# zhaoshan2/pangu-pytorch

Measured on AMD Instinct MI355X. Metric: forward steps/sec (721x1440x13pl) per MI355X, higher is better.
Workload: dtype f32; 1 GPU; PanguModel fp32 forward, 1 sample/GPU, input (1,5,13,721,1440)+(1,4,721,1440), depths 2-6-6-2, dims 192/384, random-init weights (BASELINE configs[1]); parallelism=dp1

## Files before the change

pangu-pytorch_amd/csrc/gemm_ln_f32_split.hip:

```cpp
#include "ln_epilogue_f32.h"
#include "split_f32.h"

namespace {

using namespace pangu_split;

template <int WMW, int WNW, int NST, bool ROWS, bool HAS_BIAS>
__global__ __launch_bounds__(64 * WMW * WNW, WMW * WNW == 8 ? 1 : 2) void gemm_ln_residual_f32_split_kernel(
    const float* __restrict__ A, int lda, const unsigned char* __restrict__ image, const float* __restrict__ bias,
    const float* __restrict__ shortcut, int lds_sc, const float* __restrict__ gamma, const float* __restrict__ beta,
    float* __restrict__ C, int ldc, int M, int K, float branch_scale) {
  using Tile = SplitTile<WMW, WNW, NST, ROWS>;
  __shared__ __attribute__((aligned(16))) unsigned char smem[Tile::SMEM];
  const int m0 = blockIdx.x * Tile::BM;
  f32x16 acc[Tile::RB][Tile::CB];
  split_main_loop<WMW, WNW, NST, ROWS>(smem, A, lda, image, M, Tile::BN, K, m0, 0, acc);
  if constexpr (ROWS)
    pangu_ln::ln_residual_epilogue_rows<WMW, WNW, HAS_BIAS>(smem, acc, bias, shortcut, lds_sc, gamma, beta, C, ldc, M, m0,
                                                            branch_scale);
  else
    pangu_ln::ln_residual_epilogue<WMW, WNW, HAS_BIAS, false>(smem, acc, bias, shortcut, lds_sc, gamma, beta, C, ldc, M, m0,
                                                             branch_scale);
}

template <int WMW, int WNW, int NST, bool ROWS>
int launch_ln_split(hipStream_t s, const float* A, int lda, const unsigned char* image, const float* bias, const float* shortcut,
                    int lds, const float* gamma, const float* beta, float* out, int ldo, int M, int K, float branch_scale) {
  constexpr int BM = SplitTile<WMW, WNW, NST, ROWS>::BM;
  dim3 g((M + BM - 1) / BM), blk(64 * WMW * WNW);
  if (bias)
    hipLaunchKernelGGL((gemm_ln_residual_f32_split_kernel<WMW, WNW, NST, ROWS, true>), g, blk, 0, s, A, lda, image, bias, shortcut,
                       lds, gamma, beta, out, ldo, M, K, branch_scale);
  else
    hipLaunchKernelGGL((gemm_ln_residual_f32_split_kernel<WMW, WNW, NST, ROWS, false>), g, blk, 0, s, A, lda, image, bias, shortcut,
                       lds, gamma, beta, out, ldo, M, K, branch_scale);
  return pangu_launch_status();
}

}

extern "C" int pangu_linear_ln_residual_fwd_split(pangu_stream_t stream, const float* A, int lda, const void* image,
                                                  const float* bias, const float* shortcut, int lds, const float* gamma,
                                                  const float* beta, float* out, int ldo, int M, int N, int K,
                                                  float branch_scale) {
  if (!A || !image || !shortcut || !gamma || !beta || !out) return PANGU_E_NULL;
  if (M <= 0 || K <= 0 || (K % BK) != 0 || lda < K || (lda & 3) || ldo < N || (ldo & 3) || lds < N || (lds & 3))
    return PANGU_E_SHAPE;
  if (N != 192 && N != 384) return PANGU_E_SHAPE;
  if (!pangu_fits_u32(M, lda, 4) || !pangu_fits_u32(M, ldo, 4) || !pangu_fits_u32(M, lds, 4) ||
      (long long)N * K * 6 >= 0xFFFFFFFFll)
    return PANGU_E_RANGE;
  hipStream_t s = (hipStream_t)stream;
  const unsigned char* img = reinterpret_cast<const unsigned char*>(image);
  if (N == 192) return launch_ln_split<2, 2, 3, false>(s, A, lda, img, bias, shortcut, lds, gamma, beta, out, ldo, M, K, branch_scale);
  if (K < 1536) return launch_ln_split<1, 4, 2, false>(s, A, lda, img, bias, shortcut, lds, gamma, beta, out, ldo, M, K, branch_scale);
  return launch_ln_split<2, 2, 2, true>(s, A, lda, img, bias, shortcut, lds, gamma, beta, out, ldo, M, K, branch_scale);
}
```

pangu-pytorch_amd/csrc/ln_epilogue_f32.h:

```cpp
#pragma once
#include "common.h"

namespace pangu_ln {

__device__ inline float oct_sum(float v) {
  v += __builtin_bit_cast(float, __builtin_amdgcn_update_dpp(0, __builtin_bit_cast(int, v), 0xB1, 0xF, 0xF, true));
  v += __builtin_bit_cast(float, __builtin_amdgcn_update_dpp(0, __builtin_bit_cast(int, v), 0x4E, 0xF, 0xF, true));
  v += __builtin_bit_cast(float, __builtin_amdgcn_update_dpp(0, __builtin_bit_cast(int, v), 0x141, 0xF, 0xF, true));
  return v;
}

template <int WMW, int WNW, bool HAS_BIAS, bool PIN_COL>
__device__ __forceinline__ void ln_residual_epilogue(unsigned char* smem, const f32x16 (&acc)[2][3], const float* __restrict__ bias,
                                                     const float* __restrict__ shortcut, int lds_sc,
                                                     const float* __restrict__ gamma, const float* __restrict__ beta,
                                                     float* __restrict__ C, int ldc, int M, int m0, float branch_scale) {
  constexpr int NW = WMW * WNW;
  constexpr int BN = 96 * WNW;
  constexpr int EP_LD = 36;
  constexpr float INV_C = 1.0f / BN;
  const int lane = threadIdx.x & 63;
  const int wave = __builtin_amdgcn_readfirstlane(threadIdx.x >> 6);
  const int wm = wave / WNW, wn = wave % WNW;
  const int lr = lane & 31, lh = lane >> 5;
  float* ep = reinterpret_cast<float*>(smem) + wave * (32 * EP_LD);
  float* stats = reinterpret_cast<float*>(smem) + NW * (32 * EP_LD);
  const int er = lane >> 3, ec = (lane & 7) * 4;
  const __amdgpu_buffer_rsrc_t c_rsrc = __builtin_amdgcn_make_buffer_rsrc(
      C, 0, (int)(((size_t)(M - 1) * ldc + BN) * sizeof(float)), 0x00020000);
  const __amdgpu_buffer_rsrc_t s_rsrc = __builtin_amdgcn_make_buffer_rsrc(
      const_cast<float*>(shortcut), 0, (int)(((size_t)(M - 1) * lds_sc + BN) * sizeof(float)), 0x00020000);
#pragma unroll
  for (int i = 0; i < 2; ++i) {
    f32x4 y[3][4];
    float s[4] = {0.f, 0.f, 0.f, 0.f}, q[4] = {0.f, 0.f, 0.f, 0.f};
#pragma unroll
    for (int j = 0; j < 3; ++j) {
      int col = wn * 96 + j * 32 + ec;
      if (PIN_COL) asm volatile("" : "+v"(col));
      f32x4 bv = {0.f, 0.f, 0.f, 0.f};
      if (HAS_BIAS) bv = *reinterpret_cast<const f32x4*>(bias + col);
#pragma unroll
      for (int r = 0; r < 16; ++r) ep[((r & 3) + 8 * (r >> 2) + 4 * lh) * EP_LD + lr] = acc[i][j][r];
#pragma unroll
      for (int it = 0; it < 4; ++it) {
        f32x4 v = *reinterpret_cast<const f32x4*>(&ep[(er + 8 * it) * EP_LD + ec]);
        v += bv;
        y[j][it] = v;
        s[it] += (v[0] + v[1]) + (v[2] + v[3]);
        q[it] += (v[0] * v[0] + v[1] * v[1]) + (v[2] * v[2] + v[3] * v[3]);
      }
    }
#pragma unroll
    for (int it = 0; it < 4; ++it) {
      const float ss = oct_sum(s[it]), qq = oct_sum(q[it]);
      if ((lane & 7) == 0) {
        float* st = stats + (((wm * WNW + wn) * 64) + i * 32 + er + 8 * it) * 2;
        st[0] = ss;
        st[1] = qq;
      }
    }
    __syncthreads();
    float mean[4], rstd[4];
#pragma unroll
    for (int it = 0; it < 4; ++it) {
      const int rloc = i * 32 + er + 8 * it;
      float ts = 0.f, tq = 0.f;
#pragma unroll
      for (int w = 0; w < WNW; ++w) {
        const float* st = stats + ((wm * WNW + w) * 64 + rloc) * 2;
        ts += st[0];
        tq += st[1];
      }
      mean[it] = ts * INV_C;
      rstd[it] = rsqrtf(fmaxf(tq * INV_C - mean[it] * mean[it], 0.f) + LN_EPS);
    }
#pragma unroll
    for (int j = 0; j < 3; ++j) {
      int col = wn * 96 + j * 32 + ec;
      if (PIN_COL) asm volatile("" : "+v"(col));
      const f32x4 gm = *reinterpret_cast<const f32x4*>(gamma + col);
      const f32x4 bt = *reinterpret_cast<const f32x4*>(beta + col);
#pragma unroll
      for (int it = 0; it < 4; ++it) {
        const unsigned row = (unsigned)(m0 + wm * 64 + i * 32 + er + 8 * it);
        const f32x4 sc = __builtin_bit_cast(
            f32x4, __builtin_amdgcn_raw_buffer_load_b128(s_rsrc, (int)((row * (unsigned)lds_sc + (unsigned)col) * 4u), 0, 0));
        const f32x4 v = sc + branch_scale * ((y[j][it] - mean[it]) * rstd[it] * gm + bt);
        __builtin_amdgcn_raw_buffer_store_b128(__builtin_bit_cast(u32x4, v), c_rsrc,
                                               (int)((row * (unsigned)ldc + (unsigned)col) * 4u), 0, 0);
      }
    }
  }
}

template <int WMW, int WNW, bool HAS_BIAS>
__device__ __forceinline__ void ln_residual_epilogue_rows(unsigned char* smem, const f32x16 (&acc)[1][6],
                                                          const float* __restrict__ bias, const float* __restrict__ shortcut,
                                                          int lds_sc, const float* __restrict__ gamma,
                                                          const float* __restrict__ beta, float* __restrict__ C, int ldc, int M,
                                                          int m0, float branch_scale) {
  constexpr int NW = WMW * WNW;
  constexpr int BN = 192 * WNW;
  constexpr int NG = 2 * WNW;
  constexpr int EP_LD = 36;
  constexpr float INV_C = 1.0f / BN;
  const int lane = threadIdx.x & 63;
  const int wave = __builtin_amdgcn_readfirstlane(threadIdx.x >> 6);
  const int wm = wave / WNW, wn = wave % WNW;
  const int lr = lane & 31, lh = lane >> 5;
  float* ep = reinterpret_cast<float*>(smem) + wave * (32 * EP_LD);
  float* stats = reinterpret_cast<float*>(smem) + NW * (32 * EP_LD);
  const int er = lane >> 3, ec = (lane & 7) * 4;
  const __amdgpu_buffer_rsrc_t c_rsrc = __builtin_amdgcn_make_buffer_rsrc(
      C, 0, (int)(((size_t)(M - 1) * ldc + BN) * sizeof(float)), 0x00020000);
  const __amdgpu_buffer_rsrc_t s_rsrc = __builtin_amdgcn_make_buffer_rsrc(
      const_cast<float*>(shortcut), 0, (int)(((size_t)(M - 1) * lds_sc + BN) * sizeof(float)), 0x00020000);
  f32x4 y[6][4];
#pragma unroll
  for (int g = 0; g < 2; ++g) {
    float s[4] = {0.f, 0.f, 0.f, 0.f}, q[4] = {0.f, 0.f, 0.f, 0.f};
#pragma unroll
    for (int jj = 0; jj < 3; ++jj) {
      const int j = 3 * g + jj;
      const int col = wn * 192 + j * 32 + ec;
      f32x4 bv = {0.f, 0.f, 0.f, 0.f};
      if (HAS_BIAS) bv = *reinterpret_cast<const f32x4*>(bias + col);
#pragma unroll
      for (int r = 0; r < 16; ++r) ep[((r & 3) + 8 * (r >> 2) + 4 * lh) * EP_LD + lr] = acc[0][j][r];
#pragma unroll
      for (int it = 0; it < 4; ++it) {
        f32x4 v = *reinterpret_cast<const f32x4*>(&ep[(er + 8 * it) * EP_LD + ec]);
        v += bv;
        y[j][it] = v;
        s[it] += (v[0] + v[1]) + (v[2] + v[3]);
        q[it] += (v[0] * v[0] + v[1] * v[1]) + (v[2] * v[2] + v[3] * v[3]);
      }
    }
#pragma unroll
    for (int it = 0; it < 4; ++it) {
      const float ss = oct_sum(s[it]), qq = oct_sum(q[it]);
      if ((lane & 7) == 0) {
        float* st = stats + ((wm * NG + 2 * wn + g) * 32 + er + 8 * it) * 2;
        st[0] = ss;
        st[1] = qq;
      }
    }
  }
  __syncthreads();
  float mean[4], rstd[4];
#pragma unroll
  for (int it = 0; it < 4; ++it) {
    float ts = 0.f, tq = 0.f;
#pragma unroll
    for (int g = 0; g < NG; ++g) {
      const float* st = stats + ((wm * NG + g) * 32 + er + 8 * it) * 2;
      ts += st[0];
      tq += st[1];
    }
    mean[it] = ts * INV_C;
    rstd[it] = rsqrtf(fmaxf(tq * INV_C - mean[it] * mean[it], 0.f) + LN_EPS);
  }
#pragma unroll
  for (int j = 0; j < 6; ++j) {
    const int col = wn * 192 + j * 32 + ec;
    const f32x4 gm = *reinterpret_cast<const f32x4*>(gamma + col);
    const f32x4 bt = *reinterpret_cast<const f32x4*>(beta + col);
#pragma unroll
    for (int it = 0; it < 4; ++it) {
      const unsigned row = (unsigned)(m0 + wm * 32 + er + 8 * it);
      const f32x4 sc = __builtin_bit_cast(
          f32x4, __builtin_amdgcn_raw_buffer_load_b128(s_rsrc, (int)((row * (unsigned)lds_sc + (unsigned)col) * 4u), 0, 0));
      const f32x4 v = sc + branch_scale * ((y[j][it] - mean[it]) * rstd[it] * gm + bt);
      __builtin_amdgcn_raw_buffer_store_b128(__builtin_bit_cast(u32x4, v), c_rsrc,
                                             (int)((row * (unsigned)ldc + (unsigned)col) * 4u), 0, 0);
    }
  }
}

}
```

pangu-pytorch_amd/csrc/split_f32.h:

```cpp
#pragma once
#include "gemm_f32_dma_loop.h"

namespace pangu_split {

using pangu_dma::BK;

typedef short bf16x8 __attribute__((ext_vector_type(8)));

constexpr int W_ROWS = 192;
constexpr int PLANE = 2 * W_ROWS * 16;
constexpr int B_BYTES = 3 * PLANE;
constexpr int W_PIECES = B_BYTES / 1024;

__device__ inline void split2(float a, float b, unsigned& hi, unsigned& mid, unsigned& lo) {
  const bf16x2_t h = __builtin_convertvector(f32x2_t{a, b}, bf16x2_t);
  const f32x2_t r1 = f32x2_t{a, b} - __builtin_convertvector(h, f32x2_t);
  const bf16x2_t m = __builtin_convertvector(r1, bf16x2_t);
  const f32x2_t r2 = r1 - __builtin_convertvector(m, f32x2_t);
  hi = __builtin_bit_cast(unsigned, h);
  mid = __builtin_bit_cast(unsigned, m);
  lo = __builtin_bit_cast(unsigned, __builtin_convertvector(r2, bf16x2_t));
}

__device__ inline void split8(const f32x4 c0, const f32x4 c1, bf16x8& hi, bf16x8& mid, bf16x8& lo) {
  unsigned h0, h1, h2, h3, m0, m1, m2, m3, l0, l1, l2, l3;
  split2(c0[0], c0[1], h0, m0, l0);
  split2(c0[2], c0[3], h1, m1, l1);
  split2(c1[0], c1[1], h2, m2, l2);
  split2(c1[2], c1[3], h3, m3, l3);
  hi = __builtin_bit_cast(bf16x8, u32x4{h0, h1, h2, h3});
  mid = __builtin_bit_cast(bf16x8, u32x4{m0, m1, m2, m3});
  lo = __builtin_bit_cast(bf16x8, u32x4{l0, l1, l2, l3});
}

template <int WMW, int WNW, int NST, bool ROWS>
struct SplitTile {
  static constexpr int RB = ROWS ? 1 : 2;
  static constexpr int CB = ROWS ? 6 : 3;
  static constexpr int NW = WMW * WNW;
  static constexpr int BM = 32 * RB * WMW;
  static constexpr int BN = 32 * CB * WNW;
  static constexpr int NT = BN / W_ROWS;
  static constexpr int A_BYTES = BM * 64;
  static constexpr int STAGE = A_BYTES + NT * B_BYTES;
  static constexpr int SMEM = NST * STAGE;
  static_assert(NST == 2 || NST == 3, "ring depth");
  static_assert(BN % W_ROWS == 0, "whole n-tile blocks");
};

template <int WMW, int WNW, int NST, bool ROWS, bool LEAN = false>
__device__ __forceinline__ void split_main_loop(unsigned char* smem, const float* __restrict__ A, int lda,
                                                const unsigned char* __restrict__ image, int M, int N, int K, int m0,
                                                int first_n_tile,
                                                f32x16 (&acc)[SplitTile<WMW, WNW, NST, ROWS>::RB][SplitTile<WMW, WNW, NST, ROWS>::CB]) {
  using T = SplitTile<WMW, WNW, NST, ROWS>;
  constexpr int NW = T::NW, A_BYTES = T::A_BYTES, STAGE = T::STAGE, RB = T::RB, CB = T::CB;
  constexpr int A_PIECES = A_BYTES / 1024;
  constexpr int PIECES = STAGE / 1024;
  constexpr int A_IT = A_PIECES / NW;
  constexpr int IT = (PIECES + NW - 1) / NW;
  constexpr int REM = PIECES % NW;
  static_assert(A_PIECES % NW == 0, "piece rounds");

  const int tid = threadIdx.x, lane = tid & 63;
  const int wave = __builtin_amdgcn_readfirstlane(tid >> 6);
  const int wm = wave / WNW, wn = wave % WNW;
  const int lr = lane & 31, lh = lane >> 5;
  const int KT = K / BK;

  const __amdgpu_buffer_rsrc_t a_rsrc = __builtin_amdgcn_make_buffer_rsrc(
      const_cast<float*>(A), 0, (int)(((size_t)(M - 1) * lda + K) * sizeof(float)), 0x00020000);
  const __amdgpu_buffer_rsrc_t w_rsrc = __builtin_amdgcn_make_buffer_rsrc(
      const_cast<unsigned char*>(image), 0, (int)((size_t)N * K * 6), 0x00020000);
  unsigned voff_a[A_IT], voff_w[IT - A_IT];
#pragma unroll
  for (int i = 0; i < A_IT; ++i) {
    const int row = 16 * (i * NW + wave) + (lane >> 2);
    const int f = (0x78 >> (((row >> 2) & 3) * 2)) & 3;
    voff_a[i] = ((unsigned)(m0 + row) * (unsigned)lda + ((lane & 3) ^ f) * 4) * 4u;
  }
#pragma unroll
  for (int i = A_IT; i < IT; ++i) {
    const int p = i * NW + wave - A_PIECES;
    voff_w[i - A_IT] = (unsigned)(first_n_tile + p / W_PIECES) * (unsigned)KT * (unsigned)B_BYTES +
                       (unsigned)(p % W_PIECES) * 1024u + lane * 16;
  }
  auto issue = [&](int kt, int slot) {
    unsigned char* base = smem + slot * STAGE;
#pragma unroll
    for (int i = 0; i < IT; ++i) {
      const int q = i * NW + wave;
      auto dst = (__attribute__((address_space(3))) void*)(base + q * 1024);
      if (i < A_IT) {
        __builtin_amdgcn_raw_ptr_buffer_load_lds(a_rsrc, dst, 16, (int)voff_a[i], kt * BK * 4, 0, 0);
      } else if (i * NW + NW - 1 < PIECES || q < PIECES) {
        __builtin_amdgcn_raw_ptr_buffer_load_lds(w_rsrc, dst, 16, (int)voff_w[i - A_IT], kt * B_BYTES, 0, 0);
      }
    }
  };

#pragma unroll
  for (int i = 0; i < RB; ++i)
#pragma unroll
    for (int j = 0; j < CB; ++j)
#pragma unroll
      for (int r = 0; r < 16; ++r) acc[i][j][r] = 0.f;

  int off_a[RB][2];
#pragma unroll
  for (int i = 0; i < RB; ++i)
#pragma unroll
    for (int h = 0; h < 2; ++h) off_a[i][h] = kswz64((wm * RB + i) * 32 + lr, 2 * lh + h);
  const int wcol = wn * CB * 32;
  const int off_w = A_BYTES + (wcol / W_ROWS) * B_BYTES + (lh * W_ROWS + wcol % W_ROWS + lr) * 16;

  issue(0, 0);
  if (NST == 3 && KT > 1) issue(1, 1);
  int slot = 0;
  for (int kt = 0; kt < KT; ++kt) {
    if (NST == 3 && kt + 1 < KT) {
      if (REM == 0 || wave < REM) asm volatile("s_waitcnt vmcnt(%0)" ::"n"(IT) : "memory");
      else asm volatile("s_waitcnt vmcnt(%0)" ::"n"(IT - 1) : "memory");
    } else {
      asm volatile("s_waitcnt vmcnt(0)" ::: "memory");
    }
    __builtin_amdgcn_s_barrier();
    asm volatile("" ::: "memory");
    if (NST == 3) {
      if (kt + 2 < KT) issue(kt + 2, slot == 0 ? 2 : slot - 1);
    } else {
      if (kt + 1 < KT) issue(kt + 1, slot ^ 1);
    }
    const unsigned char* St = smem + slot * STAGE;
    slot = slot == NST - 1 ? 0 : slot + 1;

    bf16x8 bw[CB][3];
    f32x4 ca[RB][2];
    auto read_w = [&](int j0, int j1) {
#pragma unroll
      for (int j = j0; j < j1; ++j)
#pragma unroll
        for (int p = 0; p < 3; ++p) bw[j][p] = *reinterpret_cast<const bf16x8*>(St + off_w + p * PLANE + j * 512);
    };
    read_w(0, LEAN ? 3 : CB);
#pragma unroll
    for (int i = 0; i < RB; ++i)
#pragma unroll
      for (int h = 0; h < 2; ++h) ca[i][h] = *reinterpret_cast<const f32x4*>(St + off_a[i][h]);
    bf16x8 ah[RB], am[RB], al[RB];
    auto tile = [&](int i, int j) {
      acc[i][j] = __builtin_amdgcn_mfma_f32_32x32x16_bf16(al[i], bw[j][0], acc[i][j], 0, 0, 0);
      acc[i][j] = __builtin_amdgcn_mfma_f32_32x32x16_bf16(ah[i], bw[j][2], acc[i][j], 0, 0, 0);
      acc[i][j] = __builtin_amdgcn_mfma_f32_32x32x16_bf16(am[i], bw[j][1], acc[i][j], 0, 0, 0);
      acc[i][j] = __builtin_amdgcn_mfma_f32_32x32x16_bf16(am[i], bw[j][0], acc[i][j], 0, 0, 0);
      acc[i][j] = __builtin_amdgcn_mfma_f32_32x32x16_bf16(ah[i], bw[j][1], acc[i][j], 0, 0, 0);
      acc[i][j] = __builtin_amdgcn_mfma_f32_32x32x16_bf16(ah[i], bw[j][0], acc[i][j], 0, 0, 0);
    };
    auto products = [&](int i) {
#pragma unroll
      for (int j = 0; j < CB; ++j) tile(i, j);
    };
    if constexpr (ROWS) {
      if constexpr (LEAN) {
        static_assert(CB == 6, "three tiles ahead");
        __builtin_amdgcn_sched_barrier(0);
        split8(ca[0][0], ca[0][1], ah[0], am[0], al[0]);
        __builtin_amdgcn_sched_barrier(0);
#pragma unroll
        for (int j = 0; j < 3; ++j) {
          tile(0, j);
          read_w(j + 3, j + 4);
          __builtin_amdgcn_sched_barrier(0);
        }
#pragma unroll
        for (int j = 3; j < CB; ++j) tile(0, j);
      } else {
        split8(ca[0][0], ca[0][1], ah[0], am[0], al[0]);
        __builtin_amdgcn_sched_group_barrier(0x100, 2 + 3 * CB, 0);
        __builtin_amdgcn_sched_group_barrier(0x002, 40, 0);
        products(0);
      }
    } else {
      static_assert(!LEAN, "LEAN is a schedule of the row-owning tiling");
      split8(ca[0][0], ca[0][1], ah[0], am[0], al[0]);
      __builtin_amdgcn_sched_barrier(0);
      products(0);
      split8(ca[1][0], ca[1][1], ah[1], am[1], al[1]);
#pragma unroll
      for (int g = 0; g < 18; ++g) {
        __builtin_amdgcn_sched_group_barrier(0x008, 1, 0);
        __builtin_amdgcn_sched_group_barrier(0x002, 3, 0);
      }
      __builtin_amdgcn_sched_barrier(0);
      products(1);
    }
  }
  __syncthreads();
}

}
```

Before: 21.93 forward steps/s.

## Prefetch residual shortcut and LN params during GEMM main loop tail

In the column-split GEMM+LayerNorm+residual kernel, the shortcut tile loads for the first 32-row half are issued inside the main loop on its second-to-last iteration. The tail waits are adjusted so those loads stay in flight while the last MFMA steps run. The second half's shortcut loads are issued before the stats barrier, and bias, gamma and beta are loaded up front. The aim is to hide global-load latency in the epilogue, at the cost of higher register pressure and hand-tuned vmcnt accounting that could hurt occupancy or correctness if misaligned.

```diff
diff --git a/pangu-pytorch_amd/csrc/gemm_ln_f32_split.hip b/pangu-pytorch_amd/csrc/gemm_ln_f32_split.hip
--- a/pangu-pytorch_amd/csrc/gemm_ln_f32_split.hip
+++ b/pangu-pytorch_amd/csrc/gemm_ln_f32_split.hip
@@ -14,13 +14,19 @@
   __shared__ __attribute__((aligned(16))) unsigned char smem[Tile::SMEM];
   const int m0 = blockIdx.x * Tile::BM;
   f32x16 acc[Tile::RB][Tile::CB];
-  split_main_loop<WMW, WNW, NST, ROWS>(smem, A, lda, image, M, Tile::BN, K, m0, 0, acc);
-  if constexpr (ROWS)
+  if constexpr (ROWS) {
+    split_main_loop<WMW, WNW, NST, ROWS>(smem, A, lda, image, M, Tile::BN, K, m0, 0, acc);
     pangu_ln::ln_residual_epilogue_rows<WMW, WNW, HAS_BIAS>(smem, acc, bias, shortcut, lds_sc, gamma, beta, C, ldc, M, m0,
                                                             branch_scale);
-  else
-    pangu_ln::ln_residual_epilogue<WMW, WNW, HAS_BIAS, false>(smem, acc, bias, shortcut, lds_sc, gamma, beta, C, ldc, M, m0,
-                                                             branch_scale);
+  } else {
+    const int wave = __builtin_amdgcn_readfirstlane(threadIdx.x >> 6);
+    const __amdgpu_buffer_rsrc_t s_rsrc = pangu_ln::shortcut_rsrc(shortcut, lds_sc, M, Tile::BN);
+    pangu_ln::ShortcutGroup first;
+    auto tail = [&]() { first.request(s_rsrc, lds_sc, m0 + (wave / WNW) * 64, (wave % WNW) * 96); };
+    split_main_loop<WMW, WNW, NST, ROWS, false, pangu_ln::ShortcutGroup::LOADS>(smem, A, lda, image, M, Tile::BN, K, m0, 0, acc, tail);
+    pangu_ln::ln_residual_epilogue<WMW, WNW, HAS_BIAS, false, true>(smem, acc, bias, shortcut, lds_sc, gamma, beta, C, ldc, M, m0,
+                                                                   branch_scale, &first);
+  }
 }
 
 template <int WMW, int WNW, int NST, bool ROWS>
diff --git a/pangu-pytorch_amd/csrc/ln_epilogue_f32.h b/pangu-pytorch_amd/csrc/ln_epilogue_f32.h
--- a/pangu-pytorch_amd/csrc/ln_epilogue_f32.h
+++ b/pangu-pytorch_amd/csrc/ln_epilogue_f32.h
@@ -10,11 +10,40 @@
   return v;
 }
 
-template <int WMW, int WNW, bool HAS_BIAS, bool PIN_COL>
+struct ShortcutGroup {
+  static constexpr int LOADS = 12;
+  f32x4 v[3][4];
+  __device__ __forceinline__ void request(__amdgpu_buffer_rsrc_t s_rsrc, int lds_sc, int row0, int col0) {
+    const int lane = threadIdx.x & 63;
+    const int er = lane >> 3, ec = (lane & 7) * 4;
+#pragma unroll
+    for (int j = 0; j < 3; ++j)
+#pragma unroll
+      for (int it = 0; it < 4; ++it) {
+        const unsigned row = (unsigned)(row0 + er + 8 * it), col = (unsigned)(col0 + j * 32 + ec);
+        v[j][it] = __builtin_bit_cast(
+            f32x4, __builtin_amdgcn_raw_buffer_load_b128(s_rsrc, (int)((row * (unsigned)lds_sc + col) * 4u), 0, 0));
+      }
+  }
+};
+
+__device__ __forceinline__ __amdgpu_buffer_rsrc_t shortcut_rsrc(const float* shortcut, int lds_sc, int M, int BN) {
+  return __builtin_amdgcn_make_buffer_rsrc(const_cast<float*>(shortcut), 0, (int)(((size_t)(M - 1) * lds_sc + BN) * sizeof(float)),
+                                           0x00020000);
+}
+
+__device__ __forceinline__ void lds_barrier() {
+  asm volatile("s_waitcnt lgkmcnt(0)" ::: "memory");
+  __builtin_amdgcn_s_barrier();
+  asm volatile("" ::: "memory");
+}
+
+template <int WMW, int WNW, bool HAS_BIAS, bool PIN_COL, bool EARLY = false>
 __device__ __forceinline__ void ln_residual_epilogue(unsigned char* smem, const f32x16 (&acc)[2][3], const float* __restrict__ bias,
                                                      const float* __restrict__ shortcut, int lds_sc,
                                                      const float* __restrict__ gamma, const float* __restrict__ beta,
-                                                     float* __restrict__ C, int ldc, int M, int m0, float branch_scale) {
+                                                     float* __restrict__ C, int ldc, int M, int m0, float branch_scale,
+                                                     const ShortcutGroup* first = nullptr) {
   constexpr int NW = WMW * WNW;
   constexpr int BN = 96 * WNW;
   constexpr int EP_LD = 36;
@@ -28,8 +57,19 @@
   const int er = lane >> 3, ec = (lane & 7) * 4;
   const __amdgpu_buffer_rsrc_t c_rsrc = __builtin_amdgcn_make_buffer_rsrc(
       C, 0, (int)(((size_t)(M - 1) * ldc + BN) * sizeof(float)), 0x00020000);
-  const __amdgpu_buffer_rsrc_t s_rsrc = __builtin_amdgcn_make_buffer_rsrc(
-      const_cast<float*>(shortcut), 0, (int)(((size_t)(M - 1) * lds_sc + BN) * sizeof(float)), 0x00020000);
+  const __amdgpu_buffer_rsrc_t s_rsrc = shortcut_rsrc(shortcut, lds_sc, M, BN);
+  ShortcutGroup sc[2];
+  f32x4 bias_[3], gm[3], bt[3];
+  if constexpr (EARLY) {
+    sc[0] = *first;
+#pragma unroll
+    for (int j = 0; j < 3; ++j) {
+      if (HAS_BIAS) bias_[j] = *reinterpret_cast<const f32x4*>(bias + wn * 96 + j * 32 + ec);
+      gm[j] = *reinterpret_cast<const f32x4*>(gamma + wn * 96 + j * 32 + ec);
+      bt[j] = *reinterpret_cast<const f32x4*>(beta + wn * 96 + j * 32 + ec);
+    }
+    asm volatile("" ::: "memory");
+  }
 #pragma unroll
   for (int i = 0; i < 2; ++i) {
     f32x4 y[3][4];
@@ -39,7 +79,7 @@
       int col = wn * 96 + j * 32 + ec;
       if (PIN_COL) asm volatile("" : "+v"(col));
       f32x4 bv = {0.f, 0.f, 0.f, 0.f};
-      if (HAS_BIAS) bv = *reinterpret_cast<const f32x4*>(bias + col);
+      if (HAS_BIAS) bv = EARLY ? bias_[j] : *reinterpret_cast<const f32x4*>(bias + col);
 #pragma unroll
       for (int r = 0; r < 16; ++r) ep[((r & 3) + 8 * (r >> 2) + 4 * lh) * EP_LD + lr] = acc[i][j][r];
 #pragma unroll
@@ -60,7 +100,12 @@
         st[1] = qq;
       }
     }
-    __syncthreads();
+    if constexpr (EARLY) {
+      if (i == 0) sc[1].request(s_rsrc, lds_sc, m0 + wm * 64 + 32, wn * 96);
+      lds_barrier();
+    } else {
+      __syncthreads();
+    }
     float mean[4], rstd[4];
 #pragma unroll
     for (int it = 0; it < 4; ++it) {
@@ -79,14 +124,18 @@
     for (int j = 0; j < 3; ++j) {
       int col = wn * 96 + j * 32 + ec;
       if (PIN_COL) asm volatile("" : "+v"(col));
-      const f32x4 gm = *reinterpret_cast<const f32x4*>(gamma + col);
-      const f32x4 bt = *reinterpret_cast<const f32x4*>(beta + col);
+      const f32x4 g4 = EARLY ? gm[j] : *reinterpret_cast<const f32x4*>(gamma + col);
+      const f32x4 b4 = EARLY ? bt[j] : *reinterpret_cast<const f32x4*>(beta + col);
 #pragma unroll
       for (int it = 0; it < 4; ++it) {
         const unsigned row = (unsigned)(m0 + wm * 64 + i * 32 + er + 8 * it);
-        const f32x4 sc = __builtin_bit_cast(
-            f32x4, __builtin_amdgcn_raw_buffer_load_b128(s_rsrc, (int)((row * (unsigned)lds_sc + (unsigned)col) * 4u), 0, 0));
-        const f32x4 v = sc + branch_scale * ((y[j][it] - mean[it]) * rstd[it] * gm + bt);
+        f32x4 s4;
+        if constexpr (EARLY)
+          s4 = sc[i].v[j][it];
+        else
+          s4 = __builtin_bit_cast(
+              f32x4, __builtin_amdgcn_raw_buffer_load_b128(s_rsrc, (int)((row * (unsigned)lds_sc + (unsigned)col) * 4u), 0, 0));
+        const f32x4 v = s4 + branch_scale * ((y[j][it] - mean[it]) * rstd[it] * g4 + b4);
         __builtin_amdgcn_raw_buffer_store_b128(__builtin_bit_cast(u32x4, v), c_rsrc,
                                                (int)((row * (unsigned)ldc + (unsigned)col) * 4u), 0, 0);
       }
diff --git a/pangu-pytorch_amd/csrc/split_f32.h b/pangu-pytorch_amd/csrc/split_f32.h
--- a/pangu-pytorch_amd/csrc/split_f32.h
+++ b/pangu-pytorch_amd/csrc/split_f32.h
@@ -48,11 +48,15 @@
   static_assert(BN % W_ROWS == 0, "whole n-tile blocks");
 };
 
-template <int WMW, int WNW, int NST, bool ROWS, bool LEAN = false>
+struct NoTail {
+  __device__ void operator()() const {}
+};
+template <int WMW, int WNW, int NST, bool ROWS, bool LEAN = false, int TAIL_LOADS = 0, class Tail = NoTail>
 __device__ __forceinline__ void split_main_loop(unsigned char* smem, const float* __restrict__ A, int lda,
                                                 const unsigned char* __restrict__ image, int M, int N, int K, int m0,
                                                 int first_n_tile,
-                                                f32x16 (&acc)[SplitTile<WMW, WNW, NST, ROWS>::RB][SplitTile<WMW, WNW, NST, ROWS>::CB]) {
+                                                f32x16 (&acc)[SplitTile<WMW, WNW, NST, ROWS>::RB][SplitTile<WMW, WNW, NST, ROWS>::CB],
+                                                Tail tail = Tail()) {
   using T = SplitTile<WMW, WNW, NST, ROWS>;
   constexpr int NW = T::NW, A_BYTES = T::A_BYTES, STAGE = T::STAGE, RB = T::RB, CB = T::CB;
   constexpr int A_PIECES = A_BYTES / 1024;
@@ -114,11 +118,22 @@
   const int wcol = wn * CB * 32;
   const int off_w = A_BYTES + (wcol / W_ROWS) * B_BYTES + (lh * W_ROWS + wcol % W_ROWS + lr) * 16;
 
+  auto issue_tail = [&]() {
+    asm volatile("" ::: "memory");
+    __builtin_amdgcn_sched_barrier(0);
+    tail();
+    asm volatile("" ::: "memory");
+    __builtin_amdgcn_sched_barrier(0);
+  };
+
   issue(0, 0);
   if (NST == 3 && KT > 1) issue(1, 1);
+  const int kt_tail = KT > 1 ? KT - 2 : 0;
   int slot = 0;
   for (int kt = 0; kt < KT; ++kt) {
-    if (NST == 3 && kt + 1 < KT) {
+    if (kt > kt_tail) {
+      asm volatile("s_waitcnt vmcnt(%0)" ::"n"(TAIL_LOADS) : "memory");
+    } else if (NST == 3 && kt + 1 < KT) {
       if (REM == 0 || wave < REM) asm volatile("s_waitcnt vmcnt(%0)" ::"n"(IT) : "memory");
       else asm volatile("s_waitcnt vmcnt(%0)" ::"n"(IT - 1) : "memory");
     } else {
@@ -131,6 +146,7 @@
     } else {
       if (kt + 1 < KT) issue(kt + 1, slot ^ 1);
     }
+    if (TAIL_LOADS > 0 && kt == kt_tail) issue_tail();
     const unsigned char* St = smem + slot * STAGE;
     slot = slot == NST - 1 ? 0 : slot + 1;
 
@@ -195,7 +211,8 @@
       products(1);
     }
   }
-  __syncthreads();
-}
-
-}
+  __builtin_amdgcn_s_barrier();
+  asm volatile("" ::: "memory");
+}
+
+}
```

Measured after the change: 22.01 forward steps/s, median of 6. About the same (+0.4%).
